# GuillaumeHolley/BloomFilterTrie

Measured on AMD Instinct MI355X. Metric: M k-mers/sec queried (presenceNode), higher is better.
Workload: dtype u64

## Files before the change

bloomfiltertrie_amd/csrc/bft_assemble.hip:

```cpp

#include <atomic>
#include <mutex>
#include <vector>

#include "bft_cs_sig.h"
#include "bft_dev.h"
#include "bft_image.h"
#include "bft_index.h"
#include "bft_scan.h"
#include "bft_sort.h"
#include "bft_walk.h"

#define ABLK 256

__global__ void k_pin_ticket(uint64_t* __restrict__ slot, uint64_t v) {
    __threadfence_system();
    *reinterpret_cast<volatile uint64_t*>(slot) = v;
}
__global__ void k_zero_words(uint32_t* __restrict__ p, uint64_t words) {
    for (uint64_t i = blockIdx.x * (uint64_t)blockDim.x + threadIdx.x; i < words; i += (uint64_t)gridDim.x * blockDim.x) p[i] = 0u;
}
int bft_zero_async(void* p, size_t bytes, hipStream_t s) {
    if (!bytes) return 0;
    if ((bytes & 3u) || ((uintptr_t)p & 3u)) return bft_fail(BFT_GPU_E_ARG, "internal: bft_zero_async wants whole aligned words");
// ... 920 lines not shown
                n += (e & BFT_CLUS_MULTI) ? (uint32_t)((e >> BFT_CLUS_LEN_SHIFT) & 0xFFFFu) : 1u;
            }
            ipos[it] = n;
        }
        __syncthreads();
        {
            const uint32_t per = (ni + FLAT_BLK - 1) / FLAT_BLK, i0 = threadIdx.x * per, i1 = i0 + per < ni ? i0 + per : ni;
            uint32_t sum = 0;
            for (uint32_t i = i0; i < i1; i++) sum += ipos[i];
            uint32_t inc = sum;
            for (int d = 1; d < 64; d <<= 1) {
                const uint32_t v = __shfl_up(inc, d);
                if ((int)lane >= d) inc += v;
            }
            if (lane == 63) wtot[wv] = inc;
            __syncthreads();
            uint32_t base = 0;
            for (uint32_t v = 0; v < wv; v++) base += wtot[v];
            uint32_t acc = base + inc - sum;
            for (uint32_t i = i0; i < i1; i++) { const uint32_t n = ipos[i]; ipos[i] = acc; acc += n; }
        }
        __syncthreads();
        for (uint32_t it = threadIdx.x; it < ni; it += FLAT_BLK) {
            const uint32_t w = it / FLAT_Q, q = it % FLAT_Q;
            const uint64_t fw = f2w[cc.f2_off + w];
            const uint64_t all = fw & ((1ull << BFT_F2_BITS_PER_WORD) - 1ull);
            uint64_t bits = (all >> (q * FLAT_QBITS)) & ((1ull << FLAT_QBITS) - 1ull);
            uint32_t clu = (uint32_t)(fw >> 48) + (uint32_t)__builtin_popcountll(all & ((1ull << (q * FLAT_QBITS)) - 1ull)), pos = ipos[it];
            for (; bits; bits &= bits - 1, clu++) {
                const uint32_t pu = w * BFT_F2_BITS_PER_WORD + q * FLAT_QBITS + (uint32_t)__builtin_ctzll(bits);
                const uint64_t e = clus[cc.clus_off + clu];
                const uint32_t len = (e & BFT_CLUS_MULTI) ? (uint32_t)((e >> BFT_CLUS_LEN_SHIFT) & 0xFFFFu) : 1u;
                for (uint32_t j = 0; j < len; j++) {
                    const uint64_t ent = (e & BFT_CLUS_MULTI) ? child[cc.child_off + (uint32_t)e + j] : e;
                    const uint32_t r = (pu << cc.s) | ((uint32_t)(ent >> BFT_CHILD_PV_SHIFT) & 0xFFu);
                    fent[cc.fent_off + pos++] = ent;
                    atomicOr((unsigned long long*)&f18[cc.f18_off + r / BFT_F2_BITS_PER_WORD], 1ull << (r % BFT_F2_BITS_PER_WORD));
                }
            }
        }
        __syncthreads();
    }
}

__global__ __launch_bounds__(ABLK) void k_flat_ranks(const BftCCX* __restrict__ ccx, uint32_t C, uint64_t* __restrict__ f18) {
    __shared__ uint32_t part[ABLK];
    const uint32_t per = (BFT_F18_WORDS + ABLK - 1) / ABLK;
    for (uint32_t c = blockIdx.x; c < C; c += gridDim.x) {
        const BftCCX cc = ccx[c];
        if (!cc.flat) continue;
        uint64_t* f = f18 + cc.f18_off;
        const uint32_t w0 = threadIdx.x * per, w1 = w0 + per < BFT_F18_WORDS ? w0 + per : BFT_F18_WORDS;
        uint32_t n = 0;
        for (uint32_t w = w0; w < w1; w++) n += (uint32_t)__builtin_popcountll(f[w]);
        part[threadIdx.x] = n;
        __syncthreads();
        if (threadIdx.x == 0) {
            uint32_t acc = 0;
            for (uint32_t i = 0; i < ABLK; i++) { const uint32_t v = part[i]; part[i] = acc; acc += v; }
        }
        __syncthreads();
        uint32_t rank = part[threadIdx.x];
        for (uint32_t w = w0; w < w1; w++) {
            const uint64_t v = f[w];
            f[w] = v | ((uint64_t)rank << 48);
            rank += (uint32_t)__builtin_popcountll(v);
        }
        __syncthreads();
    }
}


__device__ __forceinline__ uint32_t wave_list_of(uint32_t e, uint32_t a) {
    uint32_t lo = 0, hi = 63;
#pragma unroll
    for (int it = 0; it < 6; it++) {
        const uint32_t mid = (lo + hi + 1) >> 1;
        const uint32_t am = __shfl(a, mid);
        if (am <= e) lo = mid; else hi = mid - 1;
    }
    return lo;
}

__global__ __launch_bounds__(ABLK) void k_cs_sig(const uint32_t* __restrict__ seg_off, const uint32_t* __restrict__ pg, uint32_t nk, int weak, uint64_t* __restrict__ sig,
                                                 uint32_t* __restrict__ iota) {
    __shared__ unsigned long long acc[ABLK];
    const uint32_t lane = threadIdx.x & 63u, w0 = threadIdx.x & ~63u;
    const uint32_t nblk = (nk + ABLK - 1) / ABLK;
    for (uint32_t blk = blockIdx.x; blk < nblk; blk += gridDim.x) {
        const uint32_t i = blk * ABLK + threadIdx.x;
        const bool valid = i < nk;
        const uint32_t a = seg_off[valid ? i : nk], b = seg_off[valid ? i + 1 : nk];
        const uint32_t base = __shfl(a, 0), end = __shfl(b, 63);
        acc[threadIdx.x] = 0ull;
        for (uint32_t e0 = base; e0 < end; e0 += 64) {
            const uint32_t e = e0 + lane;
            const bool in = e < end;
            const uint32_t s = wave_list_of(in ? e : end - 1, a);
            if (in) atomicAdd(&acc[w0 + s], (unsigned long long)bft_cs_term(pg[e]));
        }
        if (valid) {
            sig[i] = bft_cs_finish((uint64_t)acc[threadIdx.x], b - a, weak);
            iota[i] = i;
        }
    }
}

__device__ __forceinline__ bool same_list(const uint32_t* __restrict__ seg_off, const uint32_t* __restrict__ pg, uint32_t a, uint32_t b) {
    const uint32_t la = seg_off[a + 1] - seg_off[a], lb = seg_off[b + 1] - seg_off[b];
    if (la != lb) return false;
    for (uint32_t i = 0; i < la; i++)
        if (pg[seg_off[a] + i] != pg[seg_off[b] + i]) return false;
    return true;
}


__global__ void k_cs_key2(const uint32_t* __restrict__ seg_off, const uint32_t* __restrict__ pg, uint32_t nk, int how, uint64_t* __restrict__ key2) {
    for (uint32_t i = blockIdx.x * blockDim.x + threadIdx.x; i < nk; i += gridDim.x * blockDim.x) {
        const uint32_t a = seg_off[i], b = seg_off[i + 1];
        uint64_t sum = 0;
        if (how == 0) for (uint32_t e = a; e < b; e++) sum += bft_mix64(((uint64_t)pg[e] + 1) * 0xD6E8FEB86659FD93ULL);
        if (how == 1) for (uint32_t e = a; e < b; e++) sum += bft_cs_term(pg[e]);
        key2[i] = how == 2 ? (uint64_t)(b - a) : how == 1 ? bft_cs_finish(sum, b - a, 0) : bft_mix64(sum + (uint64_t)(b - a) * 0xA24BAED4963EE407ULL);
    }
}

__global__ void k_cs_gather64(const uint64_t* __restrict__ src, const uint32_t* __restrict__ idx, uint32_t n, uint64_t* __restrict__ out) {
    for (uint32_t i = blockIdx.x * blockDim.x + threadIdx.x; i < n; i += gridDim.x * blockDim.x) out[i] = src[idx[i]];
}

__global__ void k_cs_heads(const uint64_t* __restrict__ sig_s, const uint64_t* __restrict__ key2_s, const uint32_t* __restrict__ order,
                           const uint32_t* __restrict__ seg_off, const uint32_t* __restrict__ pg, uint32_t nk, uint32_t* __restrict__ head0) {
    for (uint32_t i = blockIdx.x * blockDim.x + threadIdx.x; i < nk; i += gridDim.x * blockDim.x)
        head0[i] = (i > 0 && sig_s[i] == sig_s[i - 1] && key2_s[i] == key2_s[i - 1] && same_list(seg_off, pg, order[i], order[i - 1])) ? 0u : 1u;
}

__global__ void k_cs_headpos(const uint32_t* __restrict__ head0, const uint32_t* __restrict__ r0_ex, uint32_t nk, uint32_t* __restrict__ headpos) {
    for (uint32_t i = blockIdx.x * blockDim.x + threadIdx.x; i < nk; i += gridDim.x * blockDim.x)
        if (head0[i]) headpos[r0_ex[i]] = i;
}

__global__ void k_cs_canon(const uint64_t* __restrict__ sig_s, const uint64_t* __restrict__ key2_s, const uint32_t* __restrict__ order,
                           const uint32_t* __restrict__ head0, const uint32_t* __restrict__ r0_ex, const uint32_t* __restrict__ headpos,
                           const uint32_t* __restrict__ seg_off, const uint32_t* __restrict__ pg, uint32_t nk, uint32_t* __restrict__ canon,
                           uint32_t* __restrict__ head, uint32_t* __restrict__ len) {
    for (uint32_t i = blockIdx.x * blockDim.x + threadIdx.x; i < nk; i += gridDim.x * blockDim.x) {
        uint32_t h = 0, l = 0;
        if (head0[i]) {
            const uint32_t a = order[i];
            const uint64_t s1 = sig_s[i], s2 = key2_s[i];
            uint32_t m = i;
            for (uint32_t r = r0_ex[i]; r-- > 0;) {
                const uint32_t j = headpos[r];
                if (sig_s[j] != s1 || key2_s[j] != s2) break;
                if (same_list(seg_off, pg, a, order[j])) m = j;
            }
            canon[i] = m;
            h = m == i;
            l = h ? seg_off[a + 1] - seg_off[a] : 0;
        }
        head[i] = h;
        len[i] = l;
    }
}

__global__ void k_cs_spread(const uint32_t* __restrict__ head0, const uint32_t* __restrict__ r0_ex, const uint32_t* __restrict__ headpos, uint32_t nk,
                            uint32_t* __restrict__ canon) {
    for (uint32_t i = blockIdx.x * blockDim.x + threadIdx.x; i < nk; i += gridDim.x * blockDim.x)
        if (!head0[i]) canon[i] = canon[headpos[r0_ex[i] - 1]];
}

__global__ __launch_bounds__(ABLK) void k_cs_assign(const uint32_t* __restrict__ order, const uint32_t* __restrict__ head, const uint32_t* __restrict__ canon,
                                                    const uint32_t* __restrict__ csid_ex, const uint32_t* __restrict__ off_ex, const uint32_t* __restrict__ seg_off,
                                                    const uint32_t* __restrict__ pg, uint32_t nk, uint32_t* __restrict__ tcol, uint32_t* __restrict__ cs_off,
                                                    uint32_t* __restrict__ cs_ids) {
    const uint32_t lane = threadIdx.x & 63u;
    const uint32_t nblk = (nk + ABLK - 1) / ABLK;
    for (uint32_t blk = blockIdx.x; blk < nblk; blk += gridDim.x) {
        const uint32_t i = blk * ABLK + threadIdx.x;
        uint32_t hd = 0, src = 0, len = 0, dst = 0;
        if (i < nk) {
            const uint32_t a = order[i];
            hd = head[i];
            const uint32_t cs = csid_ex[canon[i]];
            tcol[a] = cs;
            if (hd) {
                src = seg_off[a];
                len = seg_off[a + 1] - src;
                dst = off_ex[i];
                cs_off[cs] = dst;
            }
        }
        uint64_t heads = __ballot(hd != 0);
        while (heads) {
            const int t = __builtin_ctzll(heads);
            heads &= heads - 1;
            const uint32_t s0 = __shfl(src, t), l0 = __shfl(len, t), d0 = __shfl(dst, t);
            for (uint32_t j = lane; j < l0; j += 64) cs_ids[d0 + j] = pg[s0 + j];
        }
    }
}
// ... 44 lines not shown
    __syncthreads();
    const uint32_t nblk = (nk + ABLK - 1) / ABLK;
    for (uint32_t blk = blockIdx.x; blk < nblk; blk += gridDim.x) {
        const uint32_t i = blk * ABLK + threadIdx.x;
        bool done = i >= nk;
        const unsigned long long key = done ? 0ull : cs_key(sig[i]);
        const uint32_t ch = (uint32_t)(key >> 40) & (CS_CACHE - 1u);
        uint32_t found = 0xFFFFFFFFu;
        for (int round = 0; round < 4096 && __any(!done); round++) {
            if (!done) {
                const uint32_t cand = cache[ch];
                if (cand != 0xFFFFFFFFu && tab[cand].sig == key) {
                    found = cand;
                    done = true;
                } else if (atomicCAS(&lock[ch], 0u, 1u) == 0u) {
                    uint32_t pos = (uint32_t)key & mask;
                    for (int probe = 0; probe < 64; probe++) {
                        unsigned long long cur = __hip_atomic_load(&tab[pos].sig, __ATOMIC_RELAXED, __HIP_MEMORY_SCOPE_AGENT);
                        if (cur == 0ull) {
                            cur = atomicCAS(&tab[pos].sig, 0ull, key);
                            if (cur == 0ull) {
                                tab[pos].rep = i;
                                atomicAdd(&s_new, 1u);
                                cur = key;
                            }
                        }
                        if (cur == key) { found = pos; break; }
                        pos = (pos + 1u) & mask;
                    }
                    if (found != 0xFFFFFFFFu) cache[ch] = found;
                    __threadfence_block();
                    atomicExch(&lock[ch], 0u);
                    done = true;
                }
            }
        }
        if (i < nk) {
            if (found == 0xFFFFFFFFu) atomicAdd(&s_fail, 1u);
            slot_of[i] = found;
        }
    }
    __syncthreads();
    if (threadIdx.x == 0) {
        if (s_new) atomicAdd(&counters[0], s_new);
        if (s_fail) atomicAdd(&counters[1], s_fail);
    }
}

__global__ __launch_bounds__(ABLK) void k_cs_hash_compact(const CsSlot* __restrict__ tab, uint32_t n_slots, uint64_t* __restrict__ keys, uint32_t* __restrict__ slots,
                                                          uint32_t* __restrict__ cnt) {
    __shared__ uint32_t s_cnt, s_base;
    const uint32_t per = (n_slots + gridDim.x - 1) / gridDim.x, p0 = blockIdx.x * per, p1 = min(n_slots, p0 + per);
    if (threadIdx.x == 0) s_cnt = 0;
    __syncthreads();
    uint32_t mine = 0;
    for (uint32_t p = p0 + threadIdx.x; p < p1; p += blockDim.x) mine += tab[p].sig != 0ull;
    for (int o = 32; o > 0; o >>= 1) mine += __shfl_down(mine, o);
    if ((threadIdx.x & 63u) == 0 && mine) atomicAdd(&s_cnt, mine);
    __syncthreads();
    if (threadIdx.x == 0) { s_base = s_cnt ? atomicAdd(cnt, s_cnt) : 0u; s_cnt = 0; }
    __syncthreads();
    for (uint32_t p = p0 + threadIdx.x; p < p1; p += blockDim.x) {
        const unsigned long long v = tab[p].sig;
        if (v != 0ull) {
            const uint32_t j = s_base + atomicAdd(&s_cnt, 1u);
            keys[j] = v;
            slots[j] = p;
        }
    }
}

__global__ void k_cs_hash_ids(const uint32_t* __restrict__ slots_s, uint32_t n_sets, CsSlot* __restrict__ tab, const uint32_t* __restrict__ seg_off,
                              uint32_t* __restrict__ rep, uint32_t* __restrict__ len) {
    for (uint32_t r = blockIdx.x * blockDim.x + threadIdx.x; r < n_sets; r += gridDim.x * blockDim.x) {
        CsSlot* sl = tab + slots_s[r];
        sl->id = r;
        const uint32_t a = sl->rep;
        rep[r] = a;
        len[r] = seg_off[a + 1] - seg_off[a];
    }
}

template <class T>
__global__ void k_cs_narrow(const uint32_t* __restrict__ in, uint64_t n, T* __restrict__ out) {
    for (uint64_t i = blockIdx.x * (uint64_t)blockDim.x + threadIdx.x; i < n; i += (uint64_t)gridDim.x * blockDim.x) out[i] = (T)in[i];
}

__global__ __launch_bounds__(ABLK) void k_cs_hash_copy(const uint32_t* __restrict__ rep, const uint32_t* __restrict__ cs_off, uint32_t n_sets, const uint32_t* __restrict__ seg_off,
                                                       const uint32_t* __restrict__ pg, uint32_t* __restrict__ cs_ids) {
    const uint32_t lane = threadIdx.x & 63u;
    const uint32_t nblk = (n_sets + ABLK - 1) / ABLK;
    for (uint32_t blk = blockIdx.x; blk < nblk; blk += gridDim.x) {
        const uint32_t r = blk * ABLK + threadIdx.x;
        uint32_t src = 0, len = 0, dst = 0;
        if (r < n_sets) {
            src = seg_off[rep[r]];
            dst = cs_off[r];
            len = cs_off[r + 1] - dst;
        }
        uint64_t todo = __ballot(len != 0);
        while (todo) {
            const int t = __builtin_ctzll(todo);
            todo &= todo - 1;
            const uint32_t s0 = __shfl(src, t), l0 = __shfl(len, t), d0 = __shfl(dst, t);
            for (uint32_t j = lane; j < l0; j += 64) cs_ids[d0 + j] = pg[s0 + j];
        }
    }
}

__global__ void k_cs_hash_tcol(const uint32_t* __restrict__ slot_of, const CsSlot* __restrict__ tab, uint32_t nk, uint32_t* __restrict__ tcol) {
    for (uint32_t i = blockIdx.x * blockDim.x + threadIdx.x; i < nk; i += gridDim.x * blockDim.x) tcol[i] = tab[slot_of[i]].id;
}

}

static int g_weak_signature = 0;
static unsigned long long g_exact_passes = 0, g_hash_attempts = 0;
void bft_test_weak_signature(int how) { g_weak_signature = how; }
unsigned long long bft_test_exact_passes(void) { return g_exact_passes; }

int bft_assemble_gpu(const uint64_t* d_tk, uint64_t n, int k, const uint32_t* d_hashmod, hipStream_t s, BftDeviceIndex& out, const BftAssembleHook* hook) {
    if (!bft_valid_k(k)) return bft_fail(BFT_GPU_E_ARG, "k must be in [9, 126]");
    if (n >= 0x7FFFFFFFull) return bft_fail(BFT_GPU_E_LIMIT, "more than 2^31-1 k-mers");
    switch (bft_words_for_k(k)) {
    case 1: return assemble<1>(d_tk, n, k, d_hashmod, s, out, hook);
    case 2: return assemble<2>(d_tk, n, k, d_hashmod, s, out, hook);
    case 3: return assemble<3>(d_tk, n, k, d_hashmod, s, out, hook);
    default: return assemble<4>(d_tk, n, k, d_hashmod, s, out, hook);
    }
}

int bft_flatten_gpu(const BftCC* d_ccs, uint64_t n_ccs, const uint64_t* d_f2w, const uint64_t* d_clus, const uint64_t* d_child, uint32_t flat_min,
                    hipStream_t s, DevBuf& ccx, DevBuf& f18, DevBuf& fent, uint64_t& n_f18, uint64_t& n_fent) {
    n_f18 = 0;
    n_fent = 0;
    CK(ccx.alloc(n_ccs * sizeof(BftCCX)));
    if (n_ccs == 0) {
        CK(f18.alloc(8));
        CK(fent.alloc(8));
        return 0;
    }
    const uint32_t C = (uint32_t)n_ccs;
    Scan scan(s);
    DevBuf flag, cnt, fidx, foff;
    CK(flag.alloc(n_ccs * 4));
    CK(cnt.alloc(n_ccs * 4));
    CK(fidx.alloc(n_ccs * 4));
    CK(foff.alloc(n_ccs * 4));
    const dim3 grid(bft_grid_for((n_ccs + ABLK - 1) / ABLK)), block(ABLK);
    hipLaunchKernelGGL(k_flat_flags, grid, block, 0, s, d_ccs, C, flat_min, flag.as<uint32_t>(), cnt.as<uint32_t>());
    CK(scan.enqueue(flag.as<uint32_t>(), fidx.as<uint32_t>(), n_ccs, 0));
    CK(scan.enqueue(cnt.as<uint32_t>(), foff.as<uint32_t>(), n_ccs, 1));
    CK(scan.wait());
    const uint64_t nflat = scan.get(0);
    n_fent = scan.get(1);
    n_f18 = nflat * BFT_F18_WORDS;
    if (n_f18 > 0xFFFFFFFFull) return bft_fail(BFT_GPU_E_LIMIT, "flat prefix bitmaps exceed 2^32 words");
    CK(f18.alloc_zero(n_f18 * 8, s));
    CK(fent.alloc(n_fent * 8));
    hipLaunchKernelGGL(k_ccx, grid, block, 0, s, d_ccs, flag.as<uint32_t>(), fidx.as<uint32_t>(), foff.as<uint32_t>(), C, ccx.as<BftCCX>());
    if (nflat) {
        const dim3 g2((unsigned)std::min<uint64_t>(n_ccs, 65535));
        hipLaunchKernelGGL(k_flat_fill, g2, dim3(FLAT_BLK), 0, s, ccx.as<BftCCX>(), C, d_f2w, d_clus, d_child, f18.as<uint64_t>(), fent.as<uint64_t>());
        hipLaunchKernelGGL(k_flat_ranks, g2, block, 0, s, ccx.as<BftCCX>(), C, f18.as<uint64_t>());
    }
    HIPCK(hipGetLastError());
    return 0;
}

int bft_intern_colors_gpu(const uint32_t* d_seg_off, const uint32_t* d_pg, uint64_t nk, uint64_t np, hipStream_t s, DevBuf& d_tcol,
                          DevBuf& d_cs_off, DevBuf& d_cs_ids, uint64_t& n_sets, uint64_t& n_ids, uint64_t distinct_hint, BftInternTail* tail, bool exact) {
    n_sets = 0;
    n_ids = 0;
    CK(d_tcol.alloc(nk * 4));
    if (nk == 0) {
        CK(d_cs_off.alloc_zero(4, s));
        CK(d_cs_ids.alloc(4));
        HIPCK(hipStreamSynchronize(s));
        return 0;
    }
    Scan scan(s);
    DevBuf sig, iota, bad;
    CK(iota.alloc(nk * 4));
    CK(bad.alloc(4));
    uint32_t nbad = 0;
    const dim3 grid(bft_grid_for((nk + ABLK - 1) / ABLK)), block(ABLK);
    CK(sig.alloc(nk * 8));
    hipLaunchKernelGGL(k_cs_sig, grid, block, 0, s, d_seg_off, d_pg, (uint32_t)nk, g_weak_signature ? 1 : 0, sig.as<uint64_t>(), iota.as<uint32_t>());
    bft_stage("colour sets: signatures", (double)np * 4 + (double)nk * (4 + 8 + 4), s);

    bool done = false;
    if (!exact) {
        DevBuf tab, slot_of, cnt, keys, keys_s, slots, slots_s, rep, len, tmp;
        CK(slot_of.alloc(nk * 4));
        CK(cnt.alloc(3 * 4));
        uint64_t n_slots = 1ull << 16;
        while (n_slots < nk / 8 || n_slots < 3 * distinct_hint) n_slots <<= 1;
        for (int attempt = 0; attempt < 2 && !done; attempt++) {
            if (attempt) {
                while (n_slots < 2 * nk) n_slots <<= 1;
            }
            g_hash_attempts++;
            CK(tab.alloc_zero(n_slots * sizeof(CsSlot), s));
            HIPCK(hipMemsetAsync(cnt.p, 0, 12, s));
            hipLaunchKernelGGL(k_cs_hash_insert, grid, block, 0, s, sig.as<uint64_t>(), (uint32_t)nk, tab.as<CsSlot>(), (uint32_t)(n_slots - 1), slot_of.as<uint32_t>(),
                               cnt.as<uint32_t>());
            CK(scan.publish(cnt.as<uint32_t>(), 2, 0));
            bft_stage("colour sets: hash of the signatures", (double)nk * (8 + 4) + (double)n_slots * 16, s);
            CK(scan.wait());
            if (scan.get(1) == 0 && scan.get(0) * 2 <= n_slots) done = true;
            else if (n_slots >= 2 * nk) break;
        }
        if (done) {
            n_sets = scan.get(0);
            CK(keys.alloc(n_sets * 8));
            CK(keys_s.alloc(n_sets * 8));
            CK(slots.alloc(n_sets * 4));
            CK(slots_s.alloc(n_sets * 4));
            CK(rep.alloc(n_sets * 4));
            CK(len.alloc(n_sets * 4));
            const dim3 tgrid(bft_grid_for((n_slots + ABLK - 1) / ABLK)), sgrid(bft_grid_for((n_sets + ABLK - 1) / ABLK));
            hipLaunchKernelGGL(k_cs_hash_compact, tgrid, block, 0, s, tab.as<CsSlot>(), (uint32_t)n_slots, keys.as<uint64_t>(), slots.as<uint32_t>(), cnt.as<uint32_t>() + 2);
            CK((bft_rs::sort_pairs<uint64_t, uint32_t, bft_rs::SHAPE_LIGHT>(keys.as<uint64_t>(), slots.as<uint32_t>(), n_sets, keys_s.as<uint64_t>(), slots_s.as<uint32_t>(), 0, 64, s)));
            hipLaunchKernelGGL(k_cs_hash_ids, sgrid, block, 0, s, slots_s.as<uint32_t>(), (uint32_t)n_sets, tab.as<CsSlot>(), d_seg_off, rep.as<uint32_t>(), len.as<uint32_t>());
            CK(d_cs_off.alloc((n_sets + 1) * 4));
            CK(scan.enqueue(len.as<uint32_t>(), d_cs_off.as<uint32_t>(), n_sets, 0, true));
            hipLaunchKernelGGL(k_cs_hash_tcol, grid, block, 0, s, slot_of.as<uint32_t>(), tab.as<CsSlot>(), (uint32_t)nk, d_tcol.as<uint32_t>());
            bft_stage("colour sets: distinct signatures sorted, ids, set per k-mer", (double)n_slots * 16 + (double)n_sets * (12 * 2 * 8 + 24) + (double)nk * 8, s);
            CK(scan.wait());
            n_ids = scan.get(0);
            CK(d_cs_ids.alloc(n_ids * 4));
            if (tail && tail->side && tail->pin.p &&
                (tail->done || hipEventCreateWithFlags(&tail->done, hipEventDisableTiming) == hipSuccess) &&
                (tail->ready || hipEventCreateWithFlags(&tail->ready, hipEventDisableTiming) == hipSuccess)) {
                hipStream_t t2 = tail->side;
                tail->rep.swap(rep);
                CK(tail->bad.alloc_zero(4, s));
                if (tail->narrow_w < 4) CK(tail->narrow.alloc(n_ids * tail->narrow_w));
                HIPCK(hipEventRecord(tail->ready, s));
                HIPCK(hipStreamWaitEvent(t2, tail->ready, 0));
                hipLaunchKernelGGL(k_cs_hash_copy, sgrid, block, 0, t2, tail->rep.as<uint32_t>(), d_cs_off.as<uint32_t>(), (uint32_t)n_sets, d_seg_off, d_pg, d_cs_ids.as<uint32_t>());
                hipLaunchKernelGGL(k_cs_verify, grid, block, 0, t2, d_tcol.as<uint32_t>(), d_cs_off.as<uint32_t>(), d_cs_ids.as<uint32_t>(), d_seg_off, d_pg, (uint32_t)nk,
                                   tail->bad.as<uint32_t>());
                hipLaunchKernelGGL(k_publish, dim3(1), dim3(PIN_SLOTS), 0, t2, tail->bad.as<uint32_t>(), 1, tail->pin.p);
                if (n_ids && tail->narrow_w == 1) hipLaunchKernelGGL(k_cs_narrow<uint8_t>, grid, block, 0, t2, d_cs_ids.as<uint32_t>(), n_ids, tail->narrow.as<uint8_t>());
                if (n_ids && tail->narrow_w == 2) hipLaunchKernelGGL(k_cs_narrow<uint16_t>, grid, block, 0, t2, d_cs_ids.as<uint32_t>(), n_ids, tail->narrow.as<uint16_t>());
                HIPCK(hipGetLastError());
                HIPCK(hipEventRecord(tail->done, t2));
                bft_stage("+colour sets: dictionary copied, every list verified, ids narrowed (side stream)",
                          (double)n_ids * 8 + (double)n_sets * 12 + (double)np * 8 + (double)nk * 12 + (tail->narrow_w < 4 ? (double)n_ids * (4 + tail->narrow_w) : 0.0), t2);
                tail->pending = true;
                return 0;
            }
            hipLaunchKernelGGL(k_cs_hash_copy, sgrid, block, 0, s, rep.as<uint32_t>(), d_cs_off.as<uint32_t>(), (uint32_t)n_sets, d_seg_off, d_pg, d_cs_ids.as<uint32_t>());
            bft_stage("colour sets: dictionary copied", (double)n_ids * 8 + (double)n_sets * 12, s);
            HIPCK(hipMemsetAsync(bad.p, 0, 4, s));
            hipLaunchKernelGGL(k_cs_verify, grid, block, 0, s, d_tcol.as<uint32_t>(), d_cs_off.as<uint32_t>(), d_cs_ids.as<uint32_t>(), d_seg_off, d_pg, (uint32_t)nk,
                               bad.as<uint32_t>());
            CK(scan.publish(bad.as<uint32_t>(), 1, 1));
            bft_stage("colour sets: every list verified", (double)np * 8 + (double)nk * 12, s);
            CK(scan.wait());
            nbad = (uint32_t)scan.get(1);
            done = nbad == 0;
        }
    }
    if (done) return 0;

    g_exact_passes++;
    DevBuf key2, key2_s, ord1, sig_g, sig_s, order, head0, r0, headpos, canon, head, len, csid, off;
    CK(key2.alloc(nk * 8));
    CK(key2_s.alloc(nk * 8));
    CK(ord1.alloc(nk * 4));
    CK(sig_g.alloc(nk * 8));
    CK(sig_s.alloc(nk * 8));
    CK(order.alloc(nk * 4));
    CK(head0.alloc(nk * 4));
    CK(r0.alloc(nk * 4));
    CK(headpos.alloc(nk * 4));
    CK(canon.alloc(nk * 4));
    CK(head.alloc(nk * 4));
    CK(len.alloc(nk * 4));
    CK(csid.alloc(nk * 4));
    CK(off.alloc(nk * 4));
    const uint32_t n32 = (uint32_t)nk;
    hipLaunchKernelGGL(k_cs_key2, grid, block, 0, s, d_seg_off, d_pg, n32, g_weak_signature, key2.as<uint64_t>());
    CK((bft_rs::sort_pairs<uint64_t, uint32_t, bft_rs::SHAPE_LIGHT>(key2.as<uint64_t>(), iota.as<uint32_t>(), nk, key2_s.as<uint64_t>(), ord1.as<uint32_t>(), 0, 64, s)));
    hipLaunchKernelGGL(k_cs_gather64, grid, block, 0, s, sig.as<uint64_t>(), ord1.as<uint32_t>(), n32, sig_g.as<uint64_t>());
    CK((bft_rs::sort_pairs<uint64_t, uint32_t, bft_rs::SHAPE_LIGHT>(sig_g.as<uint64_t>(), ord1.as<uint32_t>(), nk, sig_s.as<uint64_t>(), order.as<uint32_t>(), 0, 64, s)));
    hipLaunchKernelGGL(k_cs_gather64, grid, block, 0, s, key2.as<uint64_t>(), order.as<uint32_t>(), n32, key2_s.as<uint64_t>());
    hipLaunchKernelGGL(k_cs_heads, grid, block, 0, s, sig_s.as<uint64_t>(), key2_s.as<uint64_t>(), order.as<uint32_t>(), d_seg_off, d_pg, n32, head0.as<uint32_t>());
    CK(scan.run(head0.as<uint32_t>(), r0.as<uint32_t>(), nk, nullptr));
    hipLaunchKernelGGL(k_cs_headpos, grid, block, 0, s, head0.as<uint32_t>(), r0.as<uint32_t>(), n32, headpos.as<uint32_t>());
    hipLaunchKernelGGL(k_cs_canon, grid, block, 0, s, sig_s.as<uint64_t>(), key2_s.as<uint64_t>(), order.as<uint32_t>(), head0.as<uint32_t>(), r0.as<uint32_t>(),
                       headpos.as<uint32_t>(), d_seg_off, d_pg, n32, canon.as<uint32_t>(), head.as<uint32_t>(), len.as<uint32_t>());
    hipLaunchKernelGGL(k_cs_spread, grid, block, 0, s, head0.as<uint32_t>(), r0.as<uint32_t>(), headpos.as<uint32_t>(), n32, canon.as<uint32_t>());
    CK(scan.run(head.as<uint32_t>(), csid.as<uint32_t>(), nk, &n_sets));
    CK(scan.run(len.as<uint32_t>(), off.as<uint32_t>(), nk, &n_ids));
    CK(d_cs_off.alloc((n_sets + 1) * 4));
    CK(d_cs_ids.alloc(n_ids * 4));
    {
        const uint32_t t32 = (uint32_t)n_ids;
        HIPCK(hipMemcpyAsync(d_cs_off.as<uint32_t>() + n_sets, &t32, 4, hipMemcpyHostToDevice, s));
    }
    hipLaunchKernelGGL(k_cs_assign, grid, block, 0, s, order.as<uint32_t>(), head.as<uint32_t>(), canon.as<uint32_t>(), csid.as<uint32_t>(), off.as<uint32_t>(), d_seg_off,
                       d_pg, n32, d_tcol.as<uint32_t>(), d_cs_off.as<uint32_t>(), d_cs_ids.as<uint32_t>());
    HIPCK(hipMemsetAsync(bad.p, 0, 4, s));
    hipLaunchKernelGGL(k_cs_verify, grid, block, 0, s, d_tcol.as<uint32_t>(), d_cs_off.as<uint32_t>(), d_cs_ids.as<uint32_t>(), d_seg_off, d_pg, n32, bad.as<uint32_t>());
    HIPCK(hipMemcpyAsync(&nbad, bad.p, 4, hipMemcpyDeviceToHost, s));
    HIPCK(hipGetLastError());
    HIPCK(hipStreamSynchronize(s));
    if (nbad) return bft_fail(BFT_GPU_E_LIMIT, "colour-set interning self-check failed");
    (void)np;
    return 0;
}

extern "C" int bft_gpu_test_intern(const uint32_t* d_seg_off, const uint32_t* d_ids, uint64_t nk, uint64_t np, int mode, uint32_t narrow_w, uint64_t distinct_hint,
                                   uint32_t* d_tcol, uint32_t* d_cs_off, uint64_t cs_off_cap, uint32_t* d_cs_ids, uint64_t cs_ids_cap, void* d_narrow, uint64_t* counts,
                                   void* hip_stream) {
    if (!d_seg_off || !counts || (nk && (!d_tcol || !d_cs_off)) || (np && (!d_ids || !d_cs_ids))) return bft_fail(BFT_GPU_E_ARG, "NULL argument");
    if (mode < 0 || mode > 2 || (narrow_w != 1 && narrow_w != 2 && narrow_w != 4)) return bft_fail(BFT_GPU_E_ARG, "bad mode or id width");
    if (nk >= 0x7FFFFFFFull || np > 0xFFFFFFFFull) return bft_fail(BFT_GPU_E_LIMIT, "too many lists or ids");
    hipStream_t s = (hipStream_t)hip_stream;
    int dev = 0;
    HIPCK(hipGetDevice(&dev));
    bft_pool_set_stream(dev, s);
    struct Side {
        hipStream_t st = nullptr;
        ~Side() { if (st) { (void)hipStreamSynchronize(st); (void)hipStreamDestroy(st); } }
    } side;
    const unsigned long long exact0 = g_exact_passes, attempts0 = g_hash_attempts;
    DevBuf tcol, cs_off, cs_ids;
    uint64_t n_sets = 0, n_ids = 0;
    uint32_t collisions = 0;
    bool narrowed = false;
    BftInternTail tail;
    if (mode == 1) {
        HIPCK(hipStreamCreateWithFlags(&side.st, hipStreamNonBlocking));
        tail.side = side.st;
        tail.narrow_w = narrow_w;
        CK(bft_intern_colors_gpu(d_seg_off, d_ids, nk, np, s, tcol, cs_off, cs_ids, n_sets, n_ids, distinct_hint, &tail));
        CK(tail.wait(&collisions));
        if (collisions) CK(bft_intern_colors_gpu(d_seg_off, d_ids, nk, np, s, tcol, cs_off, cs_ids, n_sets, n_ids, 0, nullptr, true));
        else narrowed = narrow_w < 4 && tail.narrow.p && n_ids;
    } else {
        CK(bft_intern_colors_gpu(d_seg_off, d_ids, nk, np, s, tcol, cs_off, cs_ids, n_sets, n_ids, distinct_hint, nullptr, mode == 2));
    }
    counts[0] = n_sets;
    counts[1] = n_ids;
    counts[2] = g_exact_passes - exact0;
    counts[3] = collisions;
    counts[4] = g_hash_attempts - attempts0;
    if (n_sets + 1 > cs_off_cap || n_ids > cs_ids_cap) return bft_fail(BFT_GPU_E_NOSPACE, "dictionary does not fit the caller's arrays");
    if (nk) HIPCK(hipMemcpyAsync(d_tcol, tcol.p, nk * 4, hipMemcpyDeviceToDevice, s));
    if (nk) HIPCK(hipMemcpyAsync(d_cs_off, cs_off.p, (n_sets + 1) * 4, hipMemcpyDeviceToDevice, s));
    if (n_ids) HIPCK(hipMemcpyAsync(d_cs_ids, cs_ids.p, n_ids * 4, hipMemcpyDeviceToDevice, s));
    if (narrowed && d_narrow) HIPCK(hipMemcpyAsync(d_narrow, tail.narrow.p, n_ids * narrow_w, hipMemcpyDeviceToDevice, s));
    HIPCK(hipStreamSynchronize(s));
    return BFT_GPU_OK;
}
```

bloomfiltertrie_amd/csrc/bft_gpu.hip:

```cpp
#include <hip/hip_runtime.h>

#include <algorithm>
#include <chrono>
#include <cstring>
#include <mutex>
#include <string>
#include <thread>
#include <vector>

#include "../../include/bft_gpu.h"
#include "bft_color_plan.h"
#include "bft_file.h"
#include "bft_handle.h"
#include "bft_hash.h"
#include "bft_index.h"
#include "bft_sort.h"
#include "bft_walk.h"

#define BFT_BLOCK 256
#define BFT_ABSENT_ROW 0xFFFFFFFFu
#define BFT_MAX_GENOME_ID (1u << 24)

static thread_local std::string g_err;
int bft_fail(int code, const std::string& msg) {
// ... 1095 lines not shown
    h->log_comp = false;
    h->log_g_sorted = true;
    h->n_kmers = nk;
    h->idx_sizes[0] = idx.n_nodes * sizeof(BftNode); h->idx_sizes[1] = idx.n_bf8 * 8; h->idx_sizes[2] = idx.n_ccs * sizeof(BftCC);
    h->idx_sizes[3] = idx.n_f2w * 8; h->idx_sizes[4] = idx.n_clus * 8; h->idx_sizes[5] = idx.n_child * 8;
    h->idx_sizes[6] = idx.n_uc * (uint64_t)W * 8; h->idx_sizes[7] = idx.n_uc * 4; h->idx_sizes[8] = nk * (uint64_t)W * 8;
    h->root_ncc = (uint32_t)idx.root_ncc;
    point_image(h, std::max<uint32_t>((uint32_t)h->genomes.size(), h->any_insert ? h->max_gid_seen + 1 : 0));
    BftImage& im = h->im;

    uint64_t* I = h->info;
    I[0] = h->k;
    I[1] = nk;
    I[2] = idx.n_nodes;
    I[3] = idx.n_ccs;
    I[4] = idx.n_uc;
    I[5] = idx.n_child_nodes;
    I[6] = idx.n_prefixes;
    I[7] = idx.n_ccs_s4;
    I[8] = idx.max_ccs_per_node;
    I[9] = np;
    I[10] = img.n_sets;
    I[11] = im.nb_genomes;
    I[12] = image_bytes(h);
    I[13] = idx.root_ncc;
    I[14] = idx.root_uc;
    h->build_ms[0] = t1 - t0;
    h->build_ms[1] = t2 - t1;
    h->build_ms[2] = t3 - t2;
    h->build_ms[3] = (double)h->front_redone;
    h->built = true;
    h->claims.ensure();
    bft_trace_mark("committed (buffers released)");
    derive_root_direct(h);
    if (kh_ok) kh_adopt(h, khf, kh_ms);
    else kh_drop(h);
    if (kh_redo) derive_kmer_hash(h);
    sync_walk_kh(h);
    bft_trace_mark("root tables");
    bft_stage("root tables", 0, h->stream);
    derive_node_hash(h);
    default_launch_shape(h);
    I[12] = image_bytes(h);
    h->table_dropped = false;
    drop_table(h);
    bft_trace_mark("launch shape; done");
    bft_stage("node hash, launch shape, compact table", 0, h->stream);
    if (bft_trace_on()) {
        std::lock_guard<std::mutex> lk(g_pool_mu);
        fprintf(stderr, "[bft_gpu build] cache of released blocks: %zu blocks, %.1f MB; this process so far: %llu hipMalloc (%.2f ms), %llu hipFree on release (%.2f ms)\n", g_pool.size(),
                g_pool_bytes / 1048576.0, (unsigned long long)g_malloc_calls, g_malloc_ms, (unsigned long long)g_free_calls, g_free_ms);
    }
    h->build_ms[4] = bft_now_ms() - t3;
    return BFT_GPU_OK;
}

extern "C" int bft_gpu_build(bft_gpu* h) {
    if (!h) return fail(BFT_GPU_E_ARG, "NULL handle");
    if (h->marking) return fail(BFT_GPU_E_STATE, "build: the graph is locked for vertex marking (bft_gpu_marks_end unlocks it)");
    ENTER(h);
    if (h->built && h->log_n == 0) return BFT_GPU_OK;
    CK(wait_foreign_stream(h));
    if (h->log_comp && (!h->log_g_sorted || h->opt_no_composite)) CK(log_decompose(h));
    if (h->built) CK(bft_ensure_table(h));
    const double t0 = bft_now_ms();
    bft_trace_mark(nullptr);
    StageScope stage_scope(h);

    BftRunOut img;
    BftBuildSide side;
    BftPairRun& run = side.lists;
    CK(bft_make_run(h, run));
    bft_trace_mark("sort + dedupe done");
    bft_stage("sort + dedupe (rest)", 0, h->stream);
    const double t1 = bft_now_ms();

    img.tk.swap(run.tk);
    img.n = run.nk;
    if (img.n == 0) {
        CK(run.seg_off.alloc_zero(4, h->stream));
        CK(run.ids.alloc(4));
    }
    if (img.n > 0) (void)ensure_stream2(h);
    const bool merging = h->built && h->n_kmers > 0 && img.n > 0;
    if (img.n > 0 && !merging) kh_prepare_async(h, img.n, img.n, side.khf);
    side.tail.side = merging ? nullptr : h->stream2;
    side.tail.narrow_w = id_width(h->max_gid_seen);
    CK(bft_intern_colors_gpu(run.seg_off.as<uint32_t>(), run.ids.as<uint32_t>(), run.nk, run.np, h->stream, img.tcol, img.cs_off, img.cs_ids, img.n_sets, img.n_ids, 0, &side.tail));
    bft_trace_mark("colour sets interned");
    bft_stage("colour sets (rest)", 0, h->stream);
    if (!side.tail.pending) {
        run.seg_off.release();
        run.ids.release();
    }
    uint64_t total_pairs = run.np;
    if (merging) {
        DevBuf wide;
        const uint32_t* old_ids = nullptr;
        CK(widen_ids(h->d_cs_ids, h->n_ids, h->cs_w, h->stream, wide, &old_ids));
        const BftRun old_run{h->d_tk.as<uint64_t>(), h->d_tcol.as<uint32_t>(), h->n_kmers, h->d_cs_off.as<uint32_t>(), old_ids, h->n_sets};
        const BftRun new_run{img.tk.as<uint64_t>(), img.tcol.as<uint32_t>(), img.n, img.cs_off.as<uint32_t>(), img.cs_ids.as<uint32_t>(), img.n_sets};
        BftRunOut mo;
        CK(bft_merge_runs(h->W, old_run, new_run, h->stream, mo));
        img.swap(mo);
        CK(bft_count_pairs(img.tcol.as<uint32_t>(), img.n, img.cs_off.as<uint32_t>(), h->stream, &total_pairs));
    }
    bft_trace_mark("merge / bookkeeping");
    bft_stage("merge into the index", 0, h->stream);
    return bft_commit_image(h, img, total_pairs, t0, t1, &side);
}

int bft_ensure_built(bft_gpu* h, bool need_table) {
    if (!h->built || h->log_n) CK(bft_gpu_build(h));
    if (need_table) CK(bft_ensure_table(h));
    return 0;
}

extern "C" int bft_gpu_load_bft(const char* path, int device, bft_gpu** out) {
    if (!path || !out) return fail(BFT_GPU_E_ARG, "NULL argument");
    *out = nullptr;
    DeviceScope ds_;
    const double t_load0 = bft_now_ms();
    BftFileContent fc;
    std::string err;
    try {
        if (!bft_file_read(path, fc, err)) return fail(BFT_GPU_E_IO, err);
    } catch (const std::bad_alloc&) {
        return fail(BFT_GPU_E_IO, "out of host memory while reading the .bft file (corrupt size field?)");
    } catch (const std::exception& e) {
        return fail(BFT_GPU_E_IO, std::string("malformed .bft file: ") + e.what());
    }
    bft_gpu* h = nullptr;
    CK(bft_gpu_create_seeded(fc.k, device, fc.r1, fc.r2, &h));
    int rc = 0;
    for (const std::string& g : fc.genomes) h->genomes.push_back(g);
    const size_t B = (size_t)h->B;
    {
        uint64_t pairs = 0;
        for (const auto& v : fc.per_genome) pairs += v.size() / B;
        if (pairs && pairs <= h->opt_flush_pairs && hipSetDevice(device) == hipSuccess) {
            bft_pool_set_stream(device, h->stream);
            (void)log_reserve(h, pairs);
        }
    }
    static const bool io_trace = getenv("BFT_GPU_TRACE_IO") != nullptr;
    const double t_io0 = bft_now_ms();
    if (io_trace) fprintf(stderr, "[bft_gpu io] %8.1f ms load: file decoded, handle created, log reserved\n", t_io0 - t_load0);
    for (size_t g = 0; g < fc.per_genome.size() && rc == 0; g++)
        if (!fc.per_genome[g].empty()) rc = bft_gpu_insert_kmers(h, fc.per_genome[g].data(), fc.per_genome[g].size() / B, (uint32_t)g);
    if (io_trace) fprintf(stderr, "[bft_gpu io] %8.1f ms load: every genome's k-mers inserted (host batches)\n", bft_now_ms() - t_io0);
    if (rc == 0) rc = bft_gpu_build(h);
    if (io_trace) fprintf(stderr, "[bft_gpu io] %8.1f ms load: index built\n", bft_now_ms() - t_io0);
    bft_dispose_async(fc);
    if (rc != 0) {
        const std::string keep = g_err;
        bft_gpu_free(h);
        return fail(rc, keep);
    }
    *out = h;
    return BFT_GPU_OK;
}

template <class T, class A>
static int download(const DevBuf& d, uint64_t bytes, std::vector<T, A>& v) {
    v.resize(bytes / sizeof(T));
    if (bytes) HIPCK(hipMemcpy(v.data(), d.p, bytes, hipMemcpyDeviceToHost));
    return 0;
}
// ... 545 lines not shown
```

Baseline: 52660.

## Rework colour-set signature and dictionary copy kernels; fuse id narrowing into copy

Replaces the shared-memory atomic accumulation in the signature kernel with per-thread serial sums for short lists and whole-wave DPP reductions for long lists. The iota fill moves out of the signature kernel into the exact-path key kernel, so it is only written when the fallback runs. The dictionary copy kernel now streams lists with several loads in flight and writes the narrowed id array in the same pass, removing the separate narrow kernels. All of this is build-time colour interning work and does not touch the query path the metric measures.

```diff
diff --git a/bloomfiltertrie_amd/csrc/bft_assemble.hip b/bloomfiltertrie_amd/csrc/bft_assemble.hip
--- a/bloomfiltertrie_amd/csrc/bft_assemble.hip
+++ b/bloomfiltertrie_amd/csrc/bft_assemble.hip
@@ -1026,27 +1026,77 @@
     return lo;
 }
 
-__global__ __launch_bounds__(ABLK) void k_cs_sig(const uint32_t* __restrict__ seg_off, const uint32_t* __restrict__ pg, uint32_t nk, int weak, uint64_t* __restrict__ sig,
-                                                 uint32_t* __restrict__ iota) {
-    __shared__ unsigned long long acc[ABLK];
-    const uint32_t lane = threadIdx.x & 63u, w0 = threadIdx.x & ~63u;
+#define CS_AHEAD 4
+template <class V, class Load, class Use>
+__device__ __forceinline__ void wave_stream_lists(uint32_t a, uint32_t base_, uint32_t end_, Load load, Use use) {
+    const uint32_t lane = threadIdx.x & 63u;
+    const uint32_t base = __builtin_amdgcn_readfirstlane(base_), end = __builtin_amdgcn_readfirstlane(end_);
+    uint32_t sq[CS_AHEAD];
+    V vq[CS_AHEAD];
+    if (base >= end) return;
+    auto fetch = [&](uint64_t off, uint32_t& s, V& v) {
+        const uint32_t e = off + lane < (uint64_t)(end - base) ? base + (uint32_t)off + lane : end - 1;
+        s = wave_list_of(e, a);
+        v = load(e, s);
+    };
+#pragma unroll
+    for (uint32_t u = 0; u < CS_AHEAD; u++) fetch(64 * u, sq[u], vq[u]);
+    for (uint32_t e0 = base; e0 < end; e0 += 64) {
+#pragma unroll
+        for (uint32_t u = 0; u < CS_AHEAD; u++) {
+            if (u && (e0 += 64) >= end) break;
+            use(lane < end - e0, sq[u], vq[u]);
+            fetch((uint64_t)(e0 - base) + 64 * CS_AHEAD, sq[u], vq[u]);
+        }
+    }
+}
+
+#define CS_SHORT 8u
+
+template <int CTRL, int ROW_MASK>
+__device__ __forceinline__ uint32_t dpp_add(uint32_t v) {
+    return v + (uint32_t)__builtin_amdgcn_update_dpp(0, (int)v, CTRL, ROW_MASK, 0xf, false);
+}
+__device__ __forceinline__ uint32_t wave_sum32(uint32_t v) {
+    v = dpp_add<0xb1, 0xf>(v);
+    v = dpp_add<0x4e, 0xf>(v);
+    v = dpp_add<0x124, 0xf>(v);
+    v = dpp_add<0x128, 0xf>(v);
+    v = dpp_add<0x142, 0xa>(v);
+    v = dpp_add<0x143, 0xc>(v);
+    return (uint32_t)__builtin_amdgcn_readlane((int)v, 63);
+}
+__device__ __forceinline__ uint64_t wave_sum64(uint64_t v) {
+    const uint64_t s0 = wave_sum32((uint32_t)v & 0x3FFFFFFu), s1 = wave_sum32((uint32_t)(v >> 26) & 0x3FFFFFFu), s2 = wave_sum32((uint32_t)(v >> 52));
+    return s0 + (s1 << 26) + (s2 << 52);
+}
+
+__global__ __launch_bounds__(ABLK) void k_cs_sig(const uint32_t* __restrict__ seg_off, const uint32_t* __restrict__ pg, uint32_t nk, int weak, uint64_t* __restrict__ sig) {
+    const uint32_t lane = threadIdx.x & 63u;
     const uint32_t nblk = (nk + ABLK - 1) / ABLK;
     for (uint32_t blk = blockIdx.x; blk < nblk; blk += gridDim.x) {
         const uint32_t i = blk * ABLK + threadIdx.x;
         const bool valid = i < nk;
-        const uint32_t a = seg_off[valid ? i : nk], b = seg_off[valid ? i + 1 : nk];
-        const uint32_t base = __shfl(a, 0), end = __shfl(b, 63);
-        acc[threadIdx.x] = 0ull;
-        for (uint32_t e0 = base; e0 < end; e0 += 64) {
-            const uint32_t e = e0 + lane;
-            const bool in = e < end;
-            const uint32_t s = wave_list_of(in ? e : end - 1, a);
-            if (in) atomicAdd(&acc[w0 + s], (unsigned long long)bft_cs_term(pg[e]));
-        }
-        if (valid) {
-            sig[i] = bft_cs_finish((uint64_t)acc[threadIdx.x], b - a, weak);
-            iota[i] = i;
-        }
+        const uint32_t a = seg_off[valid ? i : nk], len = seg_off[valid ? i + 1 : nk] - a;
+        const uint32_t first = len ? pg[a] : 0u;
+        uint64_t sum = 0;
+        for (uint64_t todo = __ballot(len > CS_SHORT); todo; todo &= todo - 1) {
+            const int t = __builtin_ctzll(todo);
+            const uint32_t at = (uint32_t)__builtin_amdgcn_readlane((int)a, t), lt = (uint32_t)__builtin_amdgcn_readlane((int)len, t);
+            uint64_t part = 0;
+            for (uint32_t j0 = 0; j0 < lt; j0 += 128) {
+                const uint32_t j = j0 + lane, j1 = j + 64;
+                const uint32_t g = pg[at + (j < lt ? j : lt - 1)], g1 = pg[at + (j1 < lt ? j1 : lt - 1)];
+                part += (j < lt ? bft_cs_term(g) : 0ull) + (j1 < lt ? bft_cs_term(g1) : 0ull);
+            }
+            const uint64_t total = wave_sum64(part);
+            if (lane == (uint32_t)t) sum = total;
+        }
+        if (len && len <= CS_SHORT) {
+            sum = bft_cs_term(first);
+            for (uint32_t j = 1; j < len; j++) sum += bft_cs_term(pg[a + j]);
+        }
+        if (valid) sig[i] = bft_cs_finish(sum, len, weak);
     }
 }
 
@@ -1059,8 +1109,10 @@
 }
 
 
-__global__ void k_cs_key2(const uint32_t* __restrict__ seg_off, const uint32_t* __restrict__ pg, uint32_t nk, int how, uint64_t* __restrict__ key2) {
+__global__ void k_cs_key2(const uint32_t* __restrict__ seg_off, const uint32_t* __restrict__ pg, uint32_t nk, int how, uint64_t* __restrict__ key2,
+                          uint32_t* __restrict__ iota) {
     for (uint32_t i = blockIdx.x * blockDim.x + threadIdx.x; i < nk; i += gridDim.x * blockDim.x) {
+        iota[i] = i;
         const uint32_t a = seg_off[i], b = seg_off[i + 1];
         uint64_t sum = 0;
         if (how == 0) for (uint32_t e = a; e < b; e++) sum += bft_mix64(((uint64_t)pg[e] + 1) * 0xD6E8FEB86659FD93ULL);
@@ -1271,29 +1323,30 @@
 }
 
 template <class T>
-__global__ void k_cs_narrow(const uint32_t* __restrict__ in, uint64_t n, T* __restrict__ out) {
-    for (uint64_t i = blockIdx.x * (uint64_t)blockDim.x + threadIdx.x; i < n; i += (uint64_t)gridDim.x * blockDim.x) out[i] = (T)in[i];
-}
-
 __global__ __launch_bounds__(ABLK) void k_cs_hash_copy(const uint32_t* __restrict__ rep, const uint32_t* __restrict__ cs_off, uint32_t n_sets, const uint32_t* __restrict__ seg_off,
-                                                       const uint32_t* __restrict__ pg, uint32_t* __restrict__ cs_ids) {
+                                                       const uint32_t* __restrict__ pg, uint32_t* __restrict__ cs_ids, T* __restrict__ narrow) {
     const uint32_t lane = threadIdx.x & 63u;
     const uint32_t nblk = (n_sets + ABLK - 1) / ABLK;
     for (uint32_t blk = blockIdx.x; blk < nblk; blk += gridDim.x) {
         const uint32_t r = blk * ABLK + threadIdx.x;
-        uint32_t src = 0, len = 0, dst = 0;
-        if (r < n_sets) {
-            src = seg_off[rep[r]];
-            dst = cs_off[r];
-            len = cs_off[r + 1] - dst;
-        }
-        uint64_t todo = __ballot(len != 0);
-        while (todo) {
-            const int t = __builtin_ctzll(todo);
-            todo &= todo - 1;
-            const uint32_t s0 = __shfl(src, t), l0 = __shfl(len, t), d0 = __shfl(dst, t);
-            for (uint32_t j = lane; j < l0; j += 64) cs_ids[d0 + j] = pg[s0 + j];
-        }
+        const bool valid = r < n_sets;
+        const uint32_t a = cs_off[valid ? r : n_sets], b = cs_off[valid ? r + 1 : n_sets];
+        const uint32_t src = valid ? seg_off[rep[r]] : 0u;
+        const uint32_t base = __shfl(a, 0), end = __shfl(b, 63);
+        uint32_t d = base + lane;
+        wave_stream_lists<uint32_t>(
+            a, base, end,
+            [&](uint32_t e, uint32_t s) {
+                const uint32_t as = __shfl(a, s), srcs = __shfl(src, s);
+                return pg[srcs + (e - as)];
+            },
+            [&](bool in, uint32_t, uint32_t id) {
+                if (in) {
+                    cs_ids[d] = id;
+                    if (sizeof(T) < 4) narrow[d] = (T)id;
+                }
+                d += 64;
+            });
     }
 }
 
@@ -1357,10 +1410,19 @@
     return 0;
 }
 
+static void launch_hash_copy(dim3 grid, hipStream_t s, const uint32_t* rep, const uint32_t* cs_off, uint32_t n_sets, const uint32_t* seg_off, const uint32_t* pg,
+                             uint32_t* cs_ids, uint32_t w, void* narrow) {
+    const dim3 block(ABLK);
+    if (w == 1) hipLaunchKernelGGL(k_cs_hash_copy<uint8_t>, grid, block, 0, s, rep, cs_off, n_sets, seg_off, pg, cs_ids, (uint8_t*)narrow);
+    else if (w == 2) hipLaunchKernelGGL(k_cs_hash_copy<uint16_t>, grid, block, 0, s, rep, cs_off, n_sets, seg_off, pg, cs_ids, (uint16_t*)narrow);
+    else hipLaunchKernelGGL(k_cs_hash_copy<uint32_t>, grid, block, 0, s, rep, cs_off, n_sets, seg_off, pg, cs_ids, (uint32_t*)nullptr);
+}
+
 int bft_intern_colors_gpu(const uint32_t* d_seg_off, const uint32_t* d_pg, uint64_t nk, uint64_t np, hipStream_t s, DevBuf& d_tcol,
                           DevBuf& d_cs_off, DevBuf& d_cs_ids, uint64_t& n_sets, uint64_t& n_ids, uint64_t distinct_hint, BftInternTail* tail, bool exact) {
     n_sets = 0;
     n_ids = 0;
+    if (np > 0xFFFFFF00ull) return bft_fail(BFT_GPU_E_LIMIT, "more than 2^32 - 256 ids in the lists");
     CK(d_tcol.alloc(nk * 4));
     if (nk == 0) {
         CK(d_cs_off.alloc_zero(4, s));
@@ -1369,14 +1431,14 @@
         return 0;
     }
     Scan scan(s);
-    DevBuf sig, iota, bad;
-    CK(iota.alloc(nk * 4));
+    DevBuf sig, bad;
     CK(bad.alloc(4));
     uint32_t nbad = 0;
     const dim3 grid(bft_grid_for((nk + ABLK - 1) / ABLK)), block(ABLK);
     CK(sig.alloc(nk * 8));
-    hipLaunchKernelGGL(k_cs_sig, grid, block, 0, s, d_seg_off, d_pg, (uint32_t)nk, g_weak_signature ? 1 : 0, sig.as<uint64_t>(), iota.as<uint32_t>());
-    bft_stage("colour sets: signatures", (double)np * 4 + (double)nk * (4 + 8 + 4), s);
+    hipLaunchKernelGGL(k_cs_sig, grid, block, 0, s, d_seg_off, d_pg, (uint32_t)nk, g_weak_signature ? 1 : 0, sig.as<uint64_t>());
+    bft_trace_mark("  colour sets: signatures enqueued");
+    bft_stage("colour sets: signatures", (double)np * 4 + (double)nk * (4 + 8), s);
 
     bool done = false;
     if (!exact) {
@@ -1428,20 +1490,18 @@
                 if (tail->narrow_w < 4) CK(tail->narrow.alloc(n_ids * tail->narrow_w));
                 HIPCK(hipEventRecord(tail->ready, s));
                 HIPCK(hipStreamWaitEvent(t2, tail->ready, 0));
-                hipLaunchKernelGGL(k_cs_hash_copy, sgrid, block, 0, t2, tail->rep.as<uint32_t>(), d_cs_off.as<uint32_t>(), (uint32_t)n_sets, d_seg_off, d_pg, d_cs_ids.as<uint32_t>());
+                launch_hash_copy(sgrid, t2, tail->rep.as<uint32_t>(), d_cs_off.as<uint32_t>(), (uint32_t)n_sets, d_seg_off, d_pg, d_cs_ids.as<uint32_t>(), tail->narrow_w, tail->narrow.p);
                 hipLaunchKernelGGL(k_cs_verify, grid, block, 0, t2, d_tcol.as<uint32_t>(), d_cs_off.as<uint32_t>(), d_cs_ids.as<uint32_t>(), d_seg_off, d_pg, (uint32_t)nk,
                                    tail->bad.as<uint32_t>());
                 hipLaunchKernelGGL(k_publish, dim3(1), dim3(PIN_SLOTS), 0, t2, tail->bad.as<uint32_t>(), 1, tail->pin.p);
-                if (n_ids && tail->narrow_w == 1) hipLaunchKernelGGL(k_cs_narrow<uint8_t>, grid, block, 0, t2, d_cs_ids.as<uint32_t>(), n_ids, tail->narrow.as<uint8_t>());
-                if (n_ids && tail->narrow_w == 2) hipLaunchKernelGGL(k_cs_narrow<uint16_t>, grid, block, 0, t2, d_cs_ids.as<uint32_t>(), n_ids, tail->narrow.as<uint16_t>());
                 HIPCK(hipGetLastError());
                 HIPCK(hipEventRecord(tail->done, t2));
                 bft_stage("+colour sets: dictionary copied, every list verified, ids narrowed (side stream)",
-                          (double)n_ids * 8 + (double)n_sets * 12 + (double)np * 8 + (double)nk * 12 + (tail->narrow_w < 4 ? (double)n_ids * (4 + tail->narrow_w) : 0.0), t2);
+                          (double)n_ids * 8 + (double)n_sets * 12 + (double)np * 8 + (double)nk * 12 + (tail->narrow_w < 4 ? (double)n_ids * tail->narrow_w : 0.0), t2);
                 tail->pending = true;
                 return 0;
             }
-            hipLaunchKernelGGL(k_cs_hash_copy, sgrid, block, 0, s, rep.as<uint32_t>(), d_cs_off.as<uint32_t>(), (uint32_t)n_sets, d_seg_off, d_pg, d_cs_ids.as<uint32_t>());
+            launch_hash_copy(sgrid, s, rep.as<uint32_t>(), d_cs_off.as<uint32_t>(), (uint32_t)n_sets, d_seg_off, d_pg, d_cs_ids.as<uint32_t>(), 4, nullptr);
             bft_stage("colour sets: dictionary copied", (double)n_ids * 8 + (double)n_sets * 12, s);
             HIPCK(hipMemsetAsync(bad.p, 0, 4, s));
             hipLaunchKernelGGL(k_cs_verify, grid, block, 0, s, d_tcol.as<uint32_t>(), d_cs_off.as<uint32_t>(), d_cs_ids.as<uint32_t>(), d_seg_off, d_pg, (uint32_t)nk,
@@ -1456,8 +1516,9 @@
     if (done) return 0;
 
     g_exact_passes++;
-    DevBuf key2, key2_s, ord1, sig_g, sig_s, order, head0, r0, headpos, canon, head, len, csid, off;
+    DevBuf key2, key2_s, iota, ord1, sig_g, sig_s, order, head0, r0, headpos, canon, head, len, csid, off;
     CK(key2.alloc(nk * 8));
+    CK(iota.alloc(nk * 4));
     CK(key2_s.alloc(nk * 8));
     CK(ord1.alloc(nk * 4));
     CK(sig_g.alloc(nk * 8));
@@ -1472,7 +1533,7 @@
     CK(csid.alloc(nk * 4));
     CK(off.alloc(nk * 4));
     const uint32_t n32 = (uint32_t)nk;
-    hipLaunchKernelGGL(k_cs_key2, grid, block, 0, s, d_seg_off, d_pg, n32, g_weak_signature, key2.as<uint64_t>());
+    hipLaunchKernelGGL(k_cs_key2, grid, block, 0, s, d_seg_off, d_pg, n32, g_weak_signature, key2.as<uint64_t>(), iota.as<uint32_t>());
     CK((bft_rs::sort_pairs<uint64_t, uint32_t, bft_rs::SHAPE_LIGHT>(key2.as<uint64_t>(), iota.as<uint32_t>(), nk, key2_s.as<uint64_t>(), ord1.as<uint32_t>(), 0, 64, s)));
     hipLaunchKernelGGL(k_cs_gather64, grid, block, 0, s, sig.as<uint64_t>(), ord1.as<uint32_t>(), n32, sig_g.as<uint64_t>());
     CK((bft_rs::sort_pairs<uint64_t, uint32_t, bft_rs::SHAPE_LIGHT>(sig_g.as<uint64_t>(), ord1.as<uint32_t>(), nk, sig_s.as<uint64_t>(), order.as<uint32_t>(), 0, 64, s)));
diff --git a/bloomfiltertrie_amd/csrc/bft_gpu.hip b/bloomfiltertrie_amd/csrc/bft_gpu.hip
--- a/bloomfiltertrie_amd/csrc/bft_gpu.hip
+++ b/bloomfiltertrie_amd/csrc/bft_gpu.hip
@@ -1201,8 +1201,10 @@
         CK(run.ids.alloc(4));
     }
     if (img.n > 0) (void)ensure_stream2(h);
+    bft_trace_mark("second stream");
     const bool merging = h->built && h->n_kmers > 0 && img.n > 0;
     if (img.n > 0 && !merging) kh_prepare_async(h, img.n, img.n, side.khf);
+    bft_trace_mark("k-mer hash preparation started");
     side.tail.side = merging ? nullptr : h->stream2;
     side.tail.narrow_w = id_width(h->max_gid_seen);
     CK(bft_intern_colors_gpu(run.seg_off.as<uint32_t>(), run.ids.as<uint32_t>(), run.nk, run.np, h->stream, img.tcol, img.cs_off, img.cs_ids, img.n_sets, img.n_ids, 0, &side.tail));
```

Measured after the change: 52630. Within noise of the previous version (-0.0%).
